# maximyudayev/Realtime-ST-GCN

Hardware: AMD Instinct MI355X
Metric: skeleton-frames/sec/GPU (fwd+bwd), 10-layer ST-GCN N=64 T=300 V=25 (higher is better)
Workload: dtype bf16; 1 GPU; config 2: as_is st-gcn (fcn_in + 9 StgcnLayer, BatchNorm, Kt=9), fwd + loss + bwd + Adam; global_batch=64, seq_len=300, joints=25, parallelism=single, bn_stats=per-replica, launch=eager

## Files before the change

realtime-st-gcn_amd/csrc/conv1x1.hip:

```cpp
#include "common.h"
#include "../../include/stgcn_amd.h"
#include <stdlib.h>

namespace {

constexpr int BM = 128;
constexpr int NT = 256;

struct XGeom {
  long M;
  int ncol;
  int nrow;
  int k16n;
};

template <int KS, int BN, bool ROWB>
__global__ __launch_bounds__(NT, 2) void conv1x1_kernel(const stgcn_conv_desc a, const XGeom g) {
  constexpr int CIN = KS * 16;
  constexpr int RS = CIN * 2 + 16;
  constexpr int TM = 2, TN = BN / 64;
  constexpr int UPR = CIN / 8;
  constexpr int AU = BM * UPR / NT;
  static_assert(BM * UPR % NT == 0, "A units");
  extern __shared__ __attribute__((aligned(16))) char smem[];
  const int tid = threadIdx.x, lane = tid & 63, wave = tid >> 6;
  const int wm = wave >> 1, wn = wave & 1;
  const int lr = lane & 31, lh = lane >> 5;
  const int L = blockIdx.x, k = L >> 3;
  const int ct = k % g.ncol, rt = (k / g.ncol) * 8 + (L & 7);
  if (rt >= g.nrow) return;
  const long m0 = (long)rt * BM;
  const int n0 = ct * BN;
  const int V = a.V, S = a.stride;

  const bf16* __restrict__ in = reinterpret_cast<const bf16*>(a.in);
  {
    uint4 ra[AU];
#pragma unroll
    for (int u = 0; u < AU; ++u) {
      const int e = tid + u * NT, row = e / UPR, cu = e % UPR;
      const long m = m0 + row;
      ra[u] = make_uint4(0, 0, 0, 0);
      if (m < g.M) {
        const long fr = m / V;
        const int v = (int)(m - fr * V);
        const int t = (int)(fr % a.T_out);
        const long n = fr / a.T_out;
        int ti = -1;
        if (!a.trans) ti = t * S;
        else if (t % S == 0) ti = t / S;
        if (ti >= 0) ra[u] = *reinterpret_cast<const uint4*>(in + ((n * a.T_in + ti) * V + v) * a.in_ld + cu * 8);
      }
    }
#pragma unroll
    for (int u = 0; u < AU; ++u) {
      const int e = tid + u * NT, row = e / UPR, cu = e % UPR;
      *reinterpret_cast<uint4*>(smem + row * RS + cu * 16) = ra[u];
    }
  }
  __syncthreads();

  const bf16* __restrict__ wf = reinterpret_cast<const bf16*>(a.w_frag);
  f32x16 acc[TM][TN];
#pragma unroll
  for (int i = 0; i < TM; ++i)
#pragma unroll
    for (int j = 0; j < TN; ++j)
#pragma unroll
      for (int r = 0; r < 16; ++r) acc[i][j][r] = 0.f;
  const char* arow[TM];
#pragma unroll
  for (int i = 0; i < TM; ++i) arow[i] = smem + ((wm * TM + i) * 32 + lr) * RS + lh * 16;
  const bf16* bcol[TN];
#pragma unroll
  for (int j = 0; j < TN; ++j) bcol[j] = wf + (long)((n0 >> 5) + wn * TN + j) * g.k16n * 512 + lane * 8;
#pragma unroll
  for (int ks = 0; ks < KS; ++ks) {
    bf16x8 fb[TN], fa[TM];
#pragma unroll
    for (int j = 0; j < TN; ++j) fb[j] = __builtin_bit_cast(bf16x8, *reinterpret_cast<const uint4*>(bcol[j] + ks * 512));
#pragma unroll
    for (int i = 0; i < TM; ++i) fa[i] = __builtin_bit_cast(bf16x8, *reinterpret_cast<const uint4*>(arow[i] + ks * 32));
#pragma unroll
    for (int i = 0; i < TM; ++i)
#pragma unroll
      for (int j = 0; j < TN; ++j) acc[i][j] = __builtin_amdgcn_mfma_f32_32x32x16_bf16(fa[i], fb[j], acc[i][j], 0, 0, 0);
  }

  const int rows_valid = (int)((g.M - m0) < BM ? (g.M - m0) : BM);
  __syncthreads();
  constexpr int OS = BN * 2 + 16;
  float4* red = reinterpret_cast<float4*>(smem + BM * OS);
  int* const sbi = reinterpret_cast<int*>(smem + BM * OS + 2 * BN * 16);
  if (ROWB) {
    for (int t = tid; t < BM; t += NT) {
      const long m = m0 + (t < rows_valid ? t : 0);
      const long fr = m / V;
      const int v = (int)(m - fr * V);
      sbi[t] = a.bias_mode == 2 ? v : (int)((fr / a.T_out) * V + v);
    }
    __syncthreads();
  }
#pragma unroll
  for (int j = 0; j < TN; ++j) {
    const int cl = (wn * TN + j) * 32 + lr;
    const int col = n0 + cl;
    const float b = (!ROWB && a.bias && a.bias_mode == 1) ? a.bias[col] : 0.f;
    float s = 0.f, cnt = 0.f;
#pragma unroll
    for (int i = 0; i < TM; ++i)
#pragma unroll
      for (int r = 0; r < 16; ++r) {
        const int row = (wm * TM + i) * 32 + acc_row(r, lane);
        float bb = b;
        if (ROWB) bb = a.bias[(long)sbi[row] * a.Cout + col];
        const float v = acc[i][j][r] + bb;
        acc[i][j][r] = v;
        *reinterpret_cast<bf16*>(smem + row * OS + cl * 2) = (bf16)v;
        if (row < rows_valid) {
          s += v;
          cnt += 1.f;
        }
      }
    if (a.stats) {
      Welford w;
      w.n = cnt;
      w.mean = cnt > 0.f ? s / cnt : 0.f;
      float m2 = 0.f;
#pragma unroll
      for (int i = 0; i < TM; ++i)
#pragma unroll
        for (int r = 0; r < 16; ++r) {
          const int row = (wm * TM + i) * 32 + acc_row(r, lane);
          const float d = acc[i][j][r] - w.mean;
          if (row < rows_valid) m2 += d * d;
        }
      w.m2 = m2;
      Welford o;
      o.n = __shfl_xor(w.n, 32);
      o.mean = __shfl_xor(w.mean, 32);
      o.m2 = __shfl_xor(w.m2, 32);
      const Welford t = welford_merge(w, o);
      if (lh == 0) red[wm * BN + cl] = make_float4(t.n, t.mean, t.m2, 0.f);
    }
  }
  __syncthreads();
  if (a.stats && tid < BN) {
    const float4 p = red[tid], q = red[BN + tid];
    const Welford t = welford_merge(Welford{p.x, p.y, p.z}, Welford{q.x, q.y, q.z});
    reinterpret_cast<float4*>(a.stats)[(long)rt * a.Cout_pad + n0 + tid] = make_float4(t.n, t.mean, t.m2, 0.f);
  }
  bf16* __restrict__ out = reinterpret_cast<bf16*>(a.out);
  constexpr int OU = BN / 8;
#pragma unroll
  for (int u = 0; u < BM * OU / NT; ++u) {
    const int e = tid + u * NT, row = e / OU, cu = e % OU;
    if (row < rows_valid) {
      uint4 v = *reinterpret_cast<const uint4*>(smem + row * OS + cu * 16);
      uint4* p = reinterpret_cast<uint4*>(out + (m0 + row) * a.out_ld + n0 + cu * 8);
      if (a.accumulate) {
        float f[8], o[8];
        unpack16(v, f, (bf16*)nullptr);
        unpack16(*p, o, (bf16*)nullptr);
#pragma unroll
        for (int k = 0; k < 8; ++k) f[k] += o[k];
        v = pack16(f, (bf16*)nullptr);
      }
      *p = v;
    }
  }
}

template <bool WIDE_OUT>
__global__ __launch_bounds__(NT) void conv1x1_narrow_kernel(const stgcn_conv_desc a, long M) {
  __shared__ __attribute__((aligned(16))) float sw[4096];
  const int KP = a.Cin_pad;
  const bf16* __restrict__ w = reinterpret_cast<const bf16*>(a.w);
  for (int e = threadIdx.x; e < a.Cout_pad * KP; e += NT) sw[e] = (float)w[e];
  __syncthreads();
  const bf16* __restrict__ in = reinterpret_cast<const bf16*>(a.in);
  bf16* __restrict__ out = reinterpret_cast<bf16*>(a.out);
  const bool bias = a.bias && a.bias_mode == 1;
  if constexpr (WIDE_OUT) {
    const int CP = a.Cout_pad, CU = a.Cout / 8;
    __syncthreads();
    for (int e = threadIdx.x; e < CP * KP; e += NT) {
      const int co = e / KP, k = e - co * KP;
      sw[k * CP + co] = (float)w[e];
    }
    __syncthreads();
    const unsigned n = (unsigned)(M * CU);
    constexpr int UNR = 4;
    const bool vec_in = a.Cin <= 8 && (a.in_ld & 7) == 0 && (reinterpret_cast<size_t>(a.in) & 15) == 0;
    const unsigned gstride = gridDim.x * NT;
    for (unsigned i0 = blockIdx.x * NT + threadIdx.x; i0 < n; i0 += UNR * gstride) {
      uint4 xv[UNR];
#pragma unroll
      for (int u = 0; u < UNR; ++u) {
        const unsigned i = i0 + u * gstride;
        if (vec_in && i < n) xv[u] = *reinterpret_cast<const uint4*>(in + (long)(i / (unsigned)CU) * a.in_ld);
      }
#pragma unroll
      for (int u = 0; u < UNR; ++u) {
      const unsigned i = i0 + u * gstride;
      if (i >= n) break;
      const unsigned m = i / (unsigned)CU;
      const int c0 = (int)(i - m * (unsigned)CU) * 8;
      const bf16* xr = in + (long)m * a.in_ld;
      float xf[8];
      if (vec_in) unpack16(xv[u], xf, (bf16*)nullptr);
      float f[8];
#pragma unroll
      for (int e = 0; e < 8; ++e) f[e] = bias ? a.bias[c0 + e] : 0.f;
#pragma unroll
      for (int k = 0; k < 16; ++k)
        if (k < a.Cin) {
          const float xk = vec_in ? xf[k & 7] : (float)xr[k];
          const float4 w0 = *reinterpret_cast<const float4*>(&sw[k * CP + c0]);
          const float4 w1 = *reinterpret_cast<const float4*>(&sw[k * CP + c0 + 4]);
          f[0] = fmaf(w0.x, xk, f[0]); f[1] = fmaf(w0.y, xk, f[1]); f[2] = fmaf(w0.z, xk, f[2]); f[3] = fmaf(w0.w, xk, f[3]);
          f[4] = fmaf(w1.x, xk, f[4]); f[5] = fmaf(w1.y, xk, f[5]); f[6] = fmaf(w1.z, xk, f[6]); f[7] = fmaf(w1.w, xk, f[7]);
        }
      uint4* p = reinterpret_cast<uint4*>(out + (long)m * a.out_ld + c0);
      if (a.accumulate) {
        float o[8];
        unpack16(*p, o, (bf16*)nullptr);
#pragma unroll
        for (int e = 0; e < 8; ++e) f[e] += o[e];
      }
      *p = pack16(f, (bf16*)nullptr);
      }
    }
    return;
  }
  for (long m = (long)blockIdx.x * NT + threadIdx.x; m < M; m += (long)gridDim.x * NT) {
    float acc[8];
#pragma unroll
    for (int e = 0; e < 8; ++e) acc[e] = (bias && e < a.Cout) ? a.bias[e] : 0.f;
    uint4 xr[8];
#pragma unroll
    for (int c = 0; c < 8; ++c)
      if (c * 8 < a.Cin) xr[c] = *reinterpret_cast<const uint4*>(in + m * a.in_ld + c * 8);
#pragma unroll
    for (int c = 0; c < 8; ++c) {
      if (c * 8 >= a.Cin) break;
      const int k0 = c * 8;
      float x[8];
      unpack16(xr[c], x, (bf16*)nullptr);
#pragma unroll
      for (int e = 0; e < 8; ++e)
        if (e < a.Cout) {
#pragma unroll
          for (int k = 0; k < 8; ++k) acc[e] = fmaf(sw[e * KP + k0 + k], x[k], acc[e]);
        }
    }
    for (int k0 = 64; k0 < a.Cin; k0 += 8) {
      float x[8];
      unpack16(*reinterpret_cast<const uint4*>(in + m * a.in_ld + k0), x, (bf16*)nullptr);
#pragma unroll
      for (int e = 0; e < 8; ++e)
        if (e < a.Cout) {
#pragma unroll
          for (int k = 0; k < 8; ++k) acc[e] = fmaf(sw[e * KP + k0 + k], x[k], acc[e]);
        }
    }
#pragma unroll
    for (int e = 0; e < 8; ++e)
      if (e < a.Cout) {
        bf16* p = out + m * a.out_ld + e;
        *p = (bf16)(a.accumulate ? acc[e] + (float)*p : acc[e]);
      }
  }
}

template <int KS, int BN, bool ROWB = false>
int launch1(const stgcn_conv_desc& a, const XGeom& g, hipStream_t s) {
  constexpr int RS = KS * 16 * 2 + 16, OS = BN * 2 + 16;
  size_t lds = (size_t)BM * RS;
  const size_t lout = (size_t)BM * OS + 2 * BN * 16 + (ROWB ? BM * sizeof(int) : 0);
  if (lout > lds) lds = lout;
  constexpr bool RB = ROWB;
  if (stgcn_lds_attr((const void*)conv1x1_kernel<KS, BN, RB>, 160 * 1024, s)) return STGCN_EHIP;
  const long rounds = ((long)g.nrow + 7) / 8;
  hipLaunchKernelGGL((conv1x1_kernel<KS, BN, RB>), dim3((unsigned)(rounds * 8 * g.ncol)), dim3(NT), lds, s, a, g);
  return hipGetLastError() == hipSuccess ? STGCN_OK : STGCN_EHIP;
}

}

long conv_rows_num_row_blocks(long M, int cout);

int conv1x1_launch(const stgcn_conv_desc& a, int dtype, hipStream_t s) {
  if (dtype != 1 || a.Kt != 1 || a.pad != 0 || a.pro != 0) return -1;
  if (a.stride == 1 && a.T_in == a.T_out && !a.stats && a.bias_mode >= 0 && a.bias_mode <= 1 &&
      (long)a.Cout_pad * a.Cin_pad <= 4096) {
    const long M = (long)a.N * a.T_out * a.V;
    long nb = (M + NT - 1) / NT;
    if (nb > 1024) nb = 1024;
    if (a.Cin <= 16 && a.Cout <= 64 && a.Cout % 8 == 0 && a.out_ld % 8 == 0 && M * (a.Cout / 8) < 0x7fffffffL) {
      hipLaunchKernelGGL(conv1x1_narrow_kernel<true>, dim3((unsigned)nb), dim3(NT), 0, s, a, M);
      return hipGetLastError() == hipSuccess ? STGCN_OK : STGCN_EHIP;
    }
    if (a.Cout <= 8 && a.Cin % 8 == 0 && a.in_ld % 8 == 0) {
      hipLaunchKernelGGL(conv1x1_narrow_kernel<false>, dim3((unsigned)nb), dim3(NT), 0, s, a, M);
      return hipGetLastError() == hipSuccess ? STGCN_OK : STGCN_EHIP;
    }
  }
  if (!a.w_frag) return -1;
  if (a.stride < 1 || a.bias_mode < 0 || a.bias_mode > 3) return -1;
  if (a.bias_mode >= 2 && (a.stride != 1 || a.trans)) return -1;
  if (a.trans ? a.T_in != (a.T_out - 1) / a.stride + 1 : a.T_out != (a.T_in - 1) / a.stride + 1) return -1;
  if (a.in_ld % 8 || a.out_ld % 8 || a.Cout % 64 || a.Cin_pad != a.Cin || a.Cout_pad < a.Cout) return -1;
  if (a.Cin != 64 && a.Cin != 128 && a.Cin != 192 && a.Cin != 256) return -1;
  XGeom g;
  g.M = (long)a.N * a.T_out * a.V;
  const bool rowb = a.bias && a.bias_mode >= 2;
  const int BN = a.Cout % 128 == 0 && !rowb ? 128 : 64;
  g.ncol = a.Cout / BN;
  const long nrow = (g.M + BM - 1) / BM;
  if ((nrow + 7) / 8 * 8 * g.ncol > 0x7fffffffL) return -1;
  g.nrow = (int)nrow;
  g.k16n = a.Cin_pad / 16;
  if (a.stats && nrow > conv_rows_num_row_blocks(g.M, a.Cout)) return -1;
  if (BN == 128) {
    if (a.Cin == 64) return launch1<4, 128>(a, g, s);
    if (a.Cin == 128) return launch1<8, 128>(a, g, s);
    if (a.Cin == 192) return launch1<12, 128>(a, g, s);
    return launch1<16, 128>(a, g, s);
  }
  if (rowb) {
    if (a.Cin == 64) return launch1<4, 64, true>(a, g, s);
    if (a.Cin == 128) return launch1<8, 64, true>(a, g, s);
    if (a.Cin == 192) return launch1<12, 64, true>(a, g, s);
    return launch1<16, 64, true>(a, g, s);
  }
  if (a.Cin == 64) return launch1<4, 64>(a, g, s);
  if (a.Cin == 128) return launch1<8, 64>(a, g, s);
  if (a.Cin == 192) return launch1<12, 64>(a, g, s);
  return launch1<16, 64>(a, g, s);
}
```

realtime-st-gcn_amd/csrc/wgrad1x1.hip:

```cpp
#include "common.h"
#include "launchers.h"
#include "lds_ops.h"
#include "../../include/stgcn_amd.h"

namespace {

constexpr int NT1 = 256;
constexpr int PANEL = 32 * 64;
constexpr int GCO = 2, GCI_MAX = 8;
constexpr int TPW = GCO * GCI_MAX / 4;
constexpr int NSTAGE = 3;
constexpr int TARGET_BLOCKS = 512;

struct W1Geom {
  long steps;
  int spb;
  int nchunk;
  int ncog, ncig;
  int ncob, ncib;
  int gci;
  int pstage;
  int nstage;
};

__global__ __launch_bounds__(NT1) void wgrad1x1_kernel(const stgcn_wgrad_desc a, const W1Geom g, float* __restrict__ slab) {
  extern __shared__ __attribute__((aligned(16))) char smem[];
  const int lane = threadIdx.x & 63, wave = __builtin_amdgcn_readfirstlane(threadIdx.x >> 6);
  const int chunk = blockIdx.x, grp = blockIdx.y;
  const int gco = grp / g.ncig, gci = grp - gco * g.ncig;
  const int cob0 = gco * GCO, cib0 = gci * g.gci;
  const int nco = min(GCO, g.ncob - cob0), nci = min(g.gci, g.ncib - cib0);
  const int npan = nco + nci;
  const long s0 = (long)chunk * g.spb, s1 = min(g.steps, s0 + g.spb);
  if (s0 >= s1) return;
  const bf16* __restrict__ dy = reinterpret_cast<const bf16*>(a.dy);
  const bf16* __restrict__ x = reinterpret_cast<const bf16*>(a.in);

  const int lrow = lane >> 2, lunit = lane & 3;
  const int my_pan = (npan - wave + 3) / 4;
  const int ops = 2 * my_pan;
  auto issue = [&](long st, int stage) {
    char* base = smem + stage * g.pstage * PANEL;
    for (int p = wave; p < npan; p += 4) {
      const bf16* src;
      int ld;
      if (p < nco) {
        src = dy + (cob0 + p) * 32;
        ld = a.dy_ld;
      } else {
        src = x + (cib0 + p - nco) * 32;
        ld = a.in_ld;
      }
      const bf16* r0 = src + (st * 32 + lrow) * (long)ld + lunit * 8;
      const unsigned dst = lds_u32(base + p * PANEL);
      glds16(r0, dst);
      glds16(r0 + 16L * ld, dst + 1024);
    }
  };

  const int ntile = nco * nci;
  f32x16 acc[TPW];
#pragma unroll
  for (int k = 0; k < TPW; ++k) acc[k] = f32x16{};

  const int nst = (int)(s1 - s0);
  const int ahead = g.nstage - 1;
  for (int k = 0; k < ahead && k < nst; ++k) issue(s0 + k, k);
  int cur = 0, nxt = ahead;
  for (int si = 0; si < nst; ++si) {
    const int left = nst - 1 - si;
    wait_vm((left < ahead - 1 ? left : ahead - 1) * ops);
    asm volatile("s_waitcnt lgkmcnt(0)\n\ts_barrier" ::: "memory");
    if (si + ahead < nst) issue(s0 + si + ahead, nxt);
    nxt = nxt + 1 == g.nstage ? 0 : nxt + 1;
    const char* base = smem + cur * g.pstage * PANEL;
    cur = cur + 1 == g.nstage ? 0 : cur + 1;
#pragma unroll
    for (int k = 0; k < TPW; ++k) {
      const int t = wave + 4 * k;
      if (t >= ntile) break;
      const int cb = t / nci, ib = t - cb * nci;
      const char* pdy = base + cb * PANEL;
      const char* px = base + (nco + ib) * PANEL;
#pragma unroll
      for (int ks = 0; ks < 2; ++ks) {
        const bf16x8 fa = trfrag(pdy, 16 * ks, lane);
        const bf16x8 fb = trfrag(px, 16 * ks, lane);
        acc[k] = __builtin_amdgcn_mfma_f32_32x32x16_bf16(fa, fb, acc[k], 0, 0, 0);
      }
    }
  }
  float* part = slab + (long)chunk * a.Cout * a.Cin;
#pragma unroll
  for (int k = 0; k < TPW; ++k) {
    const int t = wave + 4 * k;
    if (t >= ntile) break;
    const int cb = t / nci, ib = t - cb * nci;
    const int ci = (cib0 + ib) * 32 + (lane & 31);
#pragma unroll
    for (int r = 0; r < 16; ++r) {
      const int co = (cob0 + cb) * 32 + acc_row(r, lane);
      part[(long)co * a.Cin + ci] = acc[k][r];
    }
  }
}

__global__ __launch_bounds__(1024) void wgrad1x1_reduce_kernel(const float* __restrict__ slab, int nchunk, long E,
                                                               float* __restrict__ dw, int overwrite) {
  __shared__ float part[16][64];
  const int le = threadIdx.x & 63, q = threadIdx.x >> 6;
  const long e = (long)blockIdx.x * 64 + le;
  float s = 0.f;
  if (e < E)
    for (int c = q; c < nchunk; c += 16) s += slab[(long)c * E + e];
  part[q][le] = s;
  __syncthreads();
  if (q != 0 || e >= E) return;
  s = 0.f;
#pragma unroll
  for (int j = 0; j < 16; ++j) s += part[j][le];
  dw[e] = overwrite ? s : dw[e] + s;
}

bool w1_ok(const stgcn_wgrad_desc& a, int dtype) {
  const long M = (long)a.N * a.T_out * a.V;
  return dtype == 1 && a.Kt == 1 && a.stride == 1 && a.pad == 0 && a.pro == 0 && a.T_in == a.T_out && M % 32 == 0 &&
         M >= 32 && a.Cin % 32 == 0 && a.Cout % 32 == 0 && a.in_ld % 8 == 0 && a.dy_ld % 8 == 0 &&
         a.in_ld >= a.Cin && a.dy_ld >= a.Cout;
}

W1Geom w1_plan(const stgcn_wgrad_desc& a) {
  W1Geom g;
  g.steps = (long)a.N * a.T_out * a.V / 32;
  g.ncob = a.Cout / 32;
  g.ncib = a.Cin / 32;
  g.gci = g.ncib <= GCI_MAX ? g.ncib : 6;
  g.ncog = (g.ncob + GCO - 1) / GCO;
  g.ncig = (g.ncib + g.gci - 1) / g.gci;
  g.pstage = (g.ncob < GCO ? g.ncob : GCO) + g.gci;
  g.nstage = (64 * 1024) / (g.pstage * PANEL);
  g.nstage = g.nstage < NSTAGE ? NSTAGE : (g.nstage > 6 ? 6 : g.nstage);
  const int groups = g.ncog * g.ncig;
  long nch = TARGET_BLOCKS / groups;
  if (nch < 1) nch = 1;
  if (nch > g.steps) nch = g.steps;
  g.spb = (int)((g.steps + nch - 1) / nch);
  g.nchunk = (int)((g.steps + g.spb - 1) / g.spb);
  return g;
}

}

long wgrad1x1_workspace(const stgcn_wgrad_desc& a, int dtype) {
  if (!w1_ok(a, dtype)) return 0;
  const W1Geom g = w1_plan(a);
  return (long)g.nchunk * a.Cout * a.Cin * (long)sizeof(float);
}

int wgrad1x1_launch(const stgcn_wgrad_desc& a, int dtype, hipStream_t s) {
  if (!w1_ok(a, dtype) || !a.work) return -1;
  const W1Geom g = w1_plan(a);
  if (a.work_bytes < (long)g.nchunk * a.Cout * a.Cin * (long)sizeof(float)) return -1;
  float* slab = reinterpret_cast<float*>(a.work);
  const size_t lds = (size_t)g.nstage * g.pstage * PANEL;
  if (stgcn_lds_attr((const void*)wgrad1x1_kernel, (int)lds, s)) return STGCN_EHIP;
  hipLaunchKernelGGL(wgrad1x1_kernel, dim3((unsigned)g.nchunk, (unsigned)(g.ncog * g.ncig)), dim3(NT1), lds, s, a, g,
                     slab);
  if (hipGetLastError() != hipSuccess) return STGCN_EHIP;
  const long E = (long)a.Cout * a.Cin;
  hipLaunchKernelGGL(wgrad1x1_reduce_kernel, dim3((unsigned)((E + 63) / 64)), dim3(1024), 0, s, (const float*)slab,
                     g.nchunk, E, a.dw, a.out_mode);
  return hipGetLastError() == hipSuccess ? STGCN_OK : STGCN_EHIP;
}
```

Before: 2.531 million skeleton-frames/s.

## Make 1x1 conv persistent with LDS-staged weights; add narrow and strided fast paths

The main 1x1 conv kernel now launches a CU-count-sized persistent grid. Each block stages its weight panel in LDS once, then loops over a contiguous run of row tiles, using a precomputed source-row table and register prefetch of the next tile's activations. A specialized register-weight path is added for the Cin<=8, Cout=64 narrow conv, and the 1x1 weight-gradient kernel now accepts strided (stride>1) inputs instead of falling back. The trade-off is more LDS per block, which may reduce occupancy, plus more complex scheduling and extra barriers per tile.

```diff
diff --git a/realtime-st-gcn_amd/csrc/conv1x1.hip b/realtime-st-gcn_amd/csrc/conv1x1.hip
--- a/realtime-st-gcn_amd/csrc/conv1x1.hip
+++ b/realtime-st-gcn_amd/csrc/conv1x1.hip
@@ -12,55 +12,116 @@
   int ncol;
   int nrow;
   int k16n;
+  int nslot;
+  int q, rem;
+  int m32;
 };
 
 template <int KS, int BN, bool ROWB>
-__global__ __launch_bounds__(NT, 2) void conv1x1_kernel(const stgcn_conv_desc a, const XGeom g) {
+struct XLds {
+  static constexpr int RS = KS * 16 * 2 + 16;
+  static constexpr int OS = BN * 2 + 16;
+  static constexpr int WB = BN * KS * 16 * 2;
+  static constexpr int OUTB = BM * OS + 2 * BN * 16 + (ROWB ? BM * (int)sizeof(int) : 0);
+  static constexpr int MAINB = BM * RS > OUTB ? BM * RS : OUTB;
+  static constexpr int TOTAL = WB + MAINB + BM * (int)sizeof(long);
+};
+
+void conv1x1_runs(int resident, XGeom* g) {
+  long cap = (resident / g->ncol) & ~7L;
+  if (cap < 8) cap = 8;
+  g->nslot = g->nrow < cap ? g->nrow : (int)cap;
+  g->q = g->nrow / g->nslot;
+  g->rem = g->nrow % g->nslot;
+}
+
+DEV long src_row(const stgcn_conv_desc& a, const XGeom& g, long m) {
+  if (m >= g.M) return -1;
+  long n;
+  int t, v;
+  if (g.m32) {
+    const unsigned um = (unsigned)m, fr = um / (unsigned)a.V, un = fr / (unsigned)a.T_out;
+    v = (int)(um - fr * (unsigned)a.V);
+    t = (int)(fr - un * (unsigned)a.T_out);
+    n = un;
+  } else {
+    const long fr = m / a.V;
+    v = (int)(m - fr * a.V);
+    n = fr / a.T_out;
+    t = (int)(fr - n * a.T_out);
+  }
+  int ti;
+  if (!a.trans) ti = t * a.stride;
+  else if (t % a.stride == 0) ti = t / a.stride;
+  else return -1;
+  return (n * a.T_in + ti) * a.V + v;
+}
+
+template <int KS, int BN, bool ROWB>
+constexpr int xbpc() { return 2 * XLds<KS, BN, ROWB>::TOTAL <= 160 * 1024 ? 2 : 1; }
+
+template <int KS, int BN, bool ROWB>
+__global__ __launch_bounds__(NT, (xbpc<KS, BN, ROWB>())) void conv1x1_kernel(const stgcn_conv_desc a, const XGeom g) {
+  typedef XLds<KS, BN, ROWB> LD;
   constexpr int CIN = KS * 16;
-  constexpr int RS = CIN * 2 + 16;
+  constexpr int RS = LD::RS;
   constexpr int TM = 2, TN = BN / 64;
   constexpr int UPR = CIN / 8;
   constexpr int AU = BM * UPR / NT;
-  static_assert(BM * UPR % NT == 0, "A units");
-  extern __shared__ __attribute__((aligned(16))) char smem[];
+  static_assert(BM * UPR % NT == 0 && AU <= 32, "A units");
+  extern __shared__ __attribute__((aligned(16))) char smem_all[];
+  char* const sw = smem_all;
+  char* const smem = smem_all + LD::WB;
+  long* const tab = reinterpret_cast<long*>(smem + LD::MAINB);
   const int tid = threadIdx.x, lane = tid & 63, wave = tid >> 6;
   const int wm = wave >> 1, wn = wave & 1;
   const int lr = lane & 31, lh = lane >> 5;
   const int L = blockIdx.x, k = L >> 3;
-  const int ct = k % g.ncol, rt = (k / g.ncol) * 8 + (L & 7);
-  if (rt >= g.nrow) return;
-  const long m0 = (long)rt * BM;
+  const int ct = k % g.ncol, slot = (k / g.ncol) * 8 + (L & 7);
+  if (slot >= g.nslot) return;
+  int rt = slot * g.q + (slot < g.rem ? slot : g.rem);
+  const int rt_end = rt + g.q + (slot < g.rem ? 1 : 0);
   const int n0 = ct * BN;
-  const int V = a.V, S = a.stride;
+  const int V = a.V;
 
   const bf16* __restrict__ in = reinterpret_cast<const bf16*>(a.in);
-  {
-    uint4 ra[AU];
+  const bf16* __restrict__ wf = reinterpret_cast<const bf16*>(a.w_frag);
+  uint4 ra[AU];
+  unsigned valid = 0;
+  auto prefetch = [&]() {
+    valid = 0;
 #pragma unroll
     for (int u = 0; u < AU; ++u) {
       const int e = tid + u * NT, row = e / UPR, cu = e % UPR;
-      const long m = m0 + row;
-      ra[u] = make_uint4(0, 0, 0, 0);
-      if (m < g.M) {
-        const long fr = m / V;
-        const int v = (int)(m - fr * V);
-        const int t = (int)(fr % a.T_out);
-        const long n = fr / a.T_out;
-        int ti = -1;
-        if (!a.trans) ti = t * S;
-        else if (t % S == 0) ti = t / S;
-        if (ti >= 0) ra[u] = *reinterpret_cast<const uint4*>(in + ((n * a.T_in + ti) * V + v) * a.in_ld + cu * 8);
-      }
-    }
-#pragma unroll
-    for (int u = 0; u < AU; ++u) {
-      const int e = tid + u * NT, row = e / UPR, cu = e % UPR;
-      *reinterpret_cast<uint4*>(smem + row * RS + cu * 16) = ra[u];
-    }
-  }
-  __syncthreads();
-
-  const bf16* __restrict__ wf = reinterpret_cast<const bf16*>(a.w_frag);
+      const long sr = tab[row];
+      valid |= (sr >= 0 ? 1u : 0u) << u;
+      ra[u] = *reinterpret_cast<const uint4*>(in + (sr >= 0 ? sr : 0) * a.in_ld + cu * 8);
+    }
+  };
+  float bcolv[TN];
+#pragma unroll
+  for (int j = 0; j < TN; ++j)
+    bcolv[j] = (!ROWB && a.bias && a.bias_mode == 1) ? a.bias[n0 + (wn * TN + j) * 32 + lr] : 0.f;
+  {
+    const uint4* src = reinterpret_cast<const uint4*>(wf + (long)(n0 >> 5) * g.k16n * 512);
+    for (int e = tid; e < LD::WB / 16; e += NT) reinterpret_cast<uint4*>(sw)[e] = src[e];
+    if (tid < BM) tab[tid] = src_row(a, g, (long)rt * BM + tid);
+    lds_barrier();
+    prefetch();
+  }
+
+  for (; rt < rt_end; ++rt) {
+  const long m0 = (long)rt * BM;
+#pragma unroll
+  for (int u = 0; u < AU; ++u) {
+    const int e = tid + u * NT, row = e / UPR, cu = e % UPR;
+    *reinterpret_cast<uint4*>(smem + row * RS + cu * 16) = (valid >> u & 1) ? ra[u] : make_uint4(0, 0, 0, 0);
+  }
+  const bool more = rt + 1 < rt_end;
+  if (more && tid < BM) tab[tid] = src_row(a, g, m0 + BM + tid);
+  lds_barrier();
+  if (more) prefetch();
+
   f32x16 acc[TM][TN];
 #pragma unroll
   for (int i = 0; i < TM; ++i)
@@ -71,14 +132,14 @@
   const char* arow[TM];
 #pragma unroll
   for (int i = 0; i < TM; ++i) arow[i] = smem + ((wm * TM + i) * 32 + lr) * RS + lh * 16;
-  const bf16* bcol[TN];
-#pragma unroll
-  for (int j = 0; j < TN; ++j) bcol[j] = wf + (long)((n0 >> 5) + wn * TN + j) * g.k16n * 512 + lane * 8;
-#pragma unroll
+  const char* bcol[TN];
+#pragma unroll
+  for (int j = 0; j < TN; ++j) bcol[j] = sw + (wn * TN + j) * KS * 1024 + lane * 16;
+#pragma unroll 4
   for (int ks = 0; ks < KS; ++ks) {
     bf16x8 fb[TN], fa[TM];
 #pragma unroll
-    for (int j = 0; j < TN; ++j) fb[j] = __builtin_bit_cast(bf16x8, *reinterpret_cast<const uint4*>(bcol[j] + ks * 512));
+    for (int j = 0; j < TN; ++j) fb[j] = __builtin_bit_cast(bf16x8, *reinterpret_cast<const uint4*>(bcol[j] + ks * 1024));
 #pragma unroll
     for (int i = 0; i < TM; ++i) fa[i] = __builtin_bit_cast(bf16x8, *reinterpret_cast<const uint4*>(arow[i] + ks * 32));
 #pragma unroll
@@ -88,8 +149,8 @@
   }
 
   const int rows_valid = (int)((g.M - m0) < BM ? (g.M - m0) : BM);
-  __syncthreads();
-  constexpr int OS = BN * 2 + 16;
+  lds_barrier();
+  constexpr int OS = LD::OS;
   float4* red = reinterpret_cast<float4*>(smem + BM * OS);
   int* const sbi = reinterpret_cast<int*>(smem + BM * OS + 2 * BN * 16);
   if (ROWB) {
@@ -99,13 +160,13 @@
       const int v = (int)(m - fr * V);
       sbi[t] = a.bias_mode == 2 ? v : (int)((fr / a.T_out) * V + v);
     }
-    __syncthreads();
+    lds_barrier();
   }
 #pragma unroll
   for (int j = 0; j < TN; ++j) {
     const int cl = (wn * TN + j) * 32 + lr;
     const int col = n0 + cl;
-    const float b = (!ROWB && a.bias && a.bias_mode == 1) ? a.bias[col] : 0.f;
+    const float b = bcolv[j];
     float s = 0.f, cnt = 0.f;
 #pragma unroll
     for (int i = 0; i < TM; ++i)
@@ -144,7 +205,7 @@
       if (lh == 0) red[wm * BN + cl] = make_float4(t.n, t.mean, t.m2, 0.f);
     }
   }
-  __syncthreads();
+  lds_barrier();
   if (a.stats && tid < BN) {
     const float4 p = red[tid], q = red[BN + tid];
     const Welford t = welford_merge(Welford{p.x, p.y, p.z}, Welford{q.x, q.y, q.z});
@@ -169,6 +230,8 @@
       *p = v;
     }
   }
+  lds_barrier();
+  }
 }
 
 template <bool WIDE_OUT>
@@ -176,11 +239,60 @@
   __shared__ __attribute__((aligned(16))) float sw[4096];
   const int KP = a.Cin_pad;
   const bf16* __restrict__ w = reinterpret_cast<const bf16*>(a.w);
-  for (int e = threadIdx.x; e < a.Cout_pad * KP; e += NT) sw[e] = (float)w[e];
-  __syncthreads();
   const bf16* __restrict__ in = reinterpret_cast<const bf16*>(a.in);
   bf16* __restrict__ out = reinterpret_cast<bf16*>(a.out);
   const bool bias = a.bias && a.bias_mode == 1;
+  if constexpr (WIDE_OUT) {
+    if (a.Cin <= 8 && a.Cout == 64 && (a.in_ld & 7) == 0 && (reinterpret_cast<size_t>(a.in) & 15) == 0 &&
+        (KP & 7) == 0 && (reinterpret_cast<size_t>(a.w) & 15) == 0) {
+      constexpr int RU = 8, RPB = NT / 8;
+      const int c0 = (threadIdx.x & 7) * 8, r = threadIdx.x >> 3;
+      float wr[8][8], bv[8];
+#pragma unroll
+      for (int e = 0; e < 8; ++e) {
+        float t[8];
+        unpack16(*reinterpret_cast<const uint4*>(w + (long)(c0 + e) * KP), t, (bf16*)nullptr);
+#pragma unroll
+        for (int k = 0; k < 8; ++k) wr[k][e] = t[k];
+        bv[e] = bias ? a.bias[c0 + e] : 0.f;
+      }
+      for (long base = (long)blockIdx.x * (RU * RPB) + r; base < M; base += (long)gridDim.x * (RU * RPB)) {
+        uint4 xv[RU];
+#pragma unroll
+        for (int u = 0; u < RU; ++u) {
+          const long m = base + u * RPB;
+          xv[u] = *reinterpret_cast<const uint4*>(in + (m < M ? m : M - 1) * a.in_ld);
+        }
+#pragma unroll
+        for (int u = 0; u < RU; ++u) {
+          const long m = base + u * RPB;
+          float xf[8], f[8];
+          unpack16(xv[u], xf, (bf16*)nullptr);
+#pragma unroll
+          for (int e = 0; e < 8; ++e) f[e] = bv[e];
+#pragma unroll
+          for (int k = 0; k < 8; ++k)
+            if (k < a.Cin) {
+#pragma unroll
+              for (int e = 0; e < 8; ++e) f[e] = fmaf(wr[k][e], xf[k], f[e]);
+            }
+          if (m < M) {
+            uint4* p = reinterpret_cast<uint4*>(out + m * a.out_ld + c0);
+            if (a.accumulate) {
+              float o[8];
+              unpack16(*p, o, (bf16*)nullptr);
+#pragma unroll
+              for (int e = 0; e < 8; ++e) f[e] += o[e];
+            }
+            *p = pack16(f, (bf16*)nullptr);
+          }
+        }
+      }
+      return;
+    }
+  }
+  for (int e = threadIdx.x; e < a.Cout_pad * KP; e += NT) sw[e] = (float)w[e];
+  __syncthreads();
   if constexpr (WIDE_OUT) {
     const int CP = a.Cout_pad, CU = a.Cout / 8;
     __syncthreads();
@@ -274,15 +386,16 @@
 }
 
 template <int KS, int BN, bool ROWB = false>
-int launch1(const stgcn_conv_desc& a, const XGeom& g, hipStream_t s) {
-  constexpr int RS = KS * 16 * 2 + 16, OS = BN * 2 + 16;
-  size_t lds = (size_t)BM * RS;
-  const size_t lout = (size_t)BM * OS + 2 * BN * 16 + (ROWB ? BM * sizeof(int) : 0);
-  if (lout > lds) lds = lout;
+int launch1(const stgcn_conv_desc& a, XGeom g, hipStream_t s) {
+  constexpr int LDS = XLds<KS, BN, ROWB>::TOTAL;
+  static_assert(LDS <= 160 * 1024, "LDS");
   constexpr bool RB = ROWB;
   if (stgcn_lds_attr((const void*)conv1x1_kernel<KS, BN, RB>, 160 * 1024, s)) return STGCN_EHIP;
-  const long rounds = ((long)g.nrow + 7) / 8;
-  hipLaunchKernelGGL((conv1x1_kernel<KS, BN, RB>), dim3((unsigned)(rounds * 8 * g.ncol)), dim3(NT), lds, s, a, g);
+  const int ncu = stgcn_cu_count(s);
+  const int bpc = xbpc<KS, BN, ROWB>();
+  conv1x1_runs((ncu > 0 ? ncu : 256) * bpc, &g);
+  const long rounds = ((long)g.nslot + 7) / 8;
+  hipLaunchKernelGGL((conv1x1_kernel<KS, BN, RB>), dim3((unsigned)(rounds * 8 * g.ncol)), dim3(NT), LDS, s, a, g);
   return hipGetLastError() == hipSuccess ? STGCN_OK : STGCN_EHIP;
 }
 
@@ -295,13 +408,17 @@
   if (a.stride == 1 && a.T_in == a.T_out && !a.stats && a.bias_mode >= 0 && a.bias_mode <= 1 &&
       (long)a.Cout_pad * a.Cin_pad <= 4096) {
     const long M = (long)a.N * a.T_out * a.V;
-    long nb = (M + NT - 1) / NT;
-    if (nb > 1024) nb = 1024;
+    const int ncu = stgcn_cu_count(s);
+    const long cap = 8L * (ncu > 0 ? ncu : 256);
     if (a.Cin <= 16 && a.Cout <= 64 && a.Cout % 8 == 0 && a.out_ld % 8 == 0 && M * (a.Cout / 8) < 0x7fffffffL) {
+      long nb = (M + 255) / 256;
+      if (nb > cap) nb = cap;
       hipLaunchKernelGGL(conv1x1_narrow_kernel<true>, dim3((unsigned)nb), dim3(NT), 0, s, a, M);
       return hipGetLastError() == hipSuccess ? STGCN_OK : STGCN_EHIP;
     }
     if (a.Cout <= 8 && a.Cin % 8 == 0 && a.in_ld % 8 == 0) {
+      long nb = (M + NT - 1) / NT;
+      if (nb > 1024) nb = 1024;
       hipLaunchKernelGGL(conv1x1_narrow_kernel<false>, dim3((unsigned)nb), dim3(NT), 0, s, a, M);
       return hipGetLastError() == hipSuccess ? STGCN_OK : STGCN_EHIP;
     }
@@ -321,6 +438,7 @@
   if ((nrow + 7) / 8 * 8 * g.ncol > 0x7fffffffL) return -1;
   g.nrow = (int)nrow;
   g.k16n = a.Cin_pad / 16;
+  g.m32 = g.M < 0x7fffffffL && (long)a.N * a.T_in * a.V < 0x7fffffffL;
   if (a.stats && nrow > conv_rows_num_row_blocks(g.M, a.Cout)) return -1;
   if (BN == 128) {
     if (a.Cin == 64) return launch1<4, 128>(a, g, s);
diff --git a/realtime-st-gcn_amd/csrc/wgrad1x1.hip b/realtime-st-gcn_amd/csrc/wgrad1x1.hip
--- a/realtime-st-gcn_amd/csrc/wgrad1x1.hip
+++ b/realtime-st-gcn_amd/csrc/wgrad1x1.hip
@@ -21,6 +21,7 @@
   int gci;
   int pstage;
   int nstage;
+  int strided;
 };
 
 __global__ __launch_bounds__(NT1) void wgrad1x1_kernel(const stgcn_wgrad_desc a, const W1Geom g, float* __restrict__ slab) {
@@ -41,20 +42,28 @@
   const int ops = 2 * my_pan;
   auto issue = [&](long st, int stage) {
     char* base = smem + stage * g.pstage * PANEL;
+    const long m0 = st * 32 + lrow, m1 = m0 + 16;
+    long x0 = m0, x1 = m1;
+    if (g.strided) {
+      const unsigned V = (unsigned)a.V, To = (unsigned)a.T_out;
+      auto xrow = [&](unsigned m) {
+        const unsigned fr = m / V, v = m - fr * V, n = fr / To, t = fr - n * To;
+        return (long)((n * (unsigned)a.T_in + t * (unsigned)a.stride) * V + v);
+      };
+      x0 = xrow((unsigned)m0);
+      x1 = xrow((unsigned)m1);
+    }
     for (int p = wave; p < npan; p += 4) {
-      const bf16* src;
-      int ld;
+      const unsigned dst = lds_u32(base + p * PANEL);
       if (p < nco) {
-        src = dy + (cob0 + p) * 32;
-        ld = a.dy_ld;
+        const bf16* src = dy + (cob0 + p) * 32 + lunit * 8;
+        glds16(src + m0 * a.dy_ld, dst);
+        glds16(src + m1 * a.dy_ld, dst + 1024);
       } else {
-        src = x + (cib0 + p - nco) * 32;
-        ld = a.in_ld;
+        const bf16* src = x + (cib0 + p - nco) * 32 + lunit * 8;
+        glds16(src + x0 * a.in_ld, dst);
+        glds16(src + x1 * a.in_ld, dst + 1024);
       }
-      const bf16* r0 = src + (st * 32 + lrow) * (long)ld + lunit * 8;
-      const unsigned dst = lds_u32(base + p * PANEL);
-      glds16(r0, dst);
-      glds16(r0 + 16L * ld, dst + 1024);
     }
   };
 
@@ -124,7 +133,9 @@
 
 bool w1_ok(const stgcn_wgrad_desc& a, int dtype) {
   const long M = (long)a.N * a.T_out * a.V;
-  return dtype == 1 && a.Kt == 1 && a.stride == 1 && a.pad == 0 && a.pro == 0 && a.T_in == a.T_out && M % 32 == 0 &&
+  if (a.stride < 1 || a.T_out < 1 || a.T_out != (a.T_in - 1) / a.stride + 1) return false;
+  if (a.stride > 1 && (M >= 0x7fffffffL || (long)a.N * a.T_in * a.V >= 0x7fffffffL)) return false;
+  return dtype == 1 && a.Kt == 1 && a.pad == 0 && a.pro == 0 && M % 32 == 0 &&
          M >= 32 && a.Cin % 32 == 0 && a.Cout % 32 == 0 && a.in_ld % 8 == 0 && a.dy_ld % 8 == 0 &&
          a.in_ld >= a.Cin && a.dy_ld >= a.Cout;
 }
@@ -132,6 +143,7 @@
 W1Geom w1_plan(const stgcn_wgrad_desc& a) {
   W1Geom g;
   g.steps = (long)a.N * a.T_out * a.V / 32;
+  g.strided = a.stride > 1;
   g.ncob = a.Cout / 32;
   g.ncib = a.Cin / 32;
   g.gci = g.ncib <= GCI_MAX ? g.ncib : 6;
```

Result: no change. 2.547 million skeleton-frames/s (median of 6 runs) (+0.6%).
